# computablelabs/starks

Measured on AMD Instinct MI355X. Metric: ntt_field_elements_per_sec, higher is better.
Workload: dtype u256 (8 x u32 limbs, integer VALU)

## Files before the change

### starks_amd/csrc/ntt.hip

```cpp
#include <stdlib.h>

#include <atomic>

#include "knobs.hpp"
#include "ntt_kernels.cuh"

namespace {

template <int LOG_R, bool LAST, int TILE_LOG>
hipError_t launch_tile(const NttPassArgs& a, bool xcd, hipStream_t st) {
  constexpr int LOG_T = TILE_LOG - LOG_R;
  static std::atomic<uint64_t> attr_done{0};
  return shk_launch_tile_kernel(ntt_pass_kernel<LOG_R, LOG_T, LAST>, attr_done, LOG_T, 1u << (TILE_LOG - 2), (size_t)32 << TILE_LOG,
                                a, xcd, st);
}

template <int LOG_R, bool LAST, int TILE_LOG>
hipError_t launch_narrow(const NttPassArgs& a, hipStream_t st) {
  constexpr int LOG_T = TILE_LOG - LOG_R;
  const uint64_t tiles = (a.total + ((1ull << LOG_T) - 1)) >> LOG_T;
  if (tiles == 0 || tiles > 0x7ffffff0ull) return hipErrorInvalidValue;
  hipLaunchKernelGGL((ntt_narrow_pass_kernel<LOG_R, LOG_T, LAST>), dim3((unsigned)tiles), dim3(1u << (TILE_LOG - 1)), 0, st, a);
  return hipGetLastError();
}

template <int LOG_R, bool LAST>
hipError_t launch_cell(const ShkNttCell& c, const NttPassArgs& a, hipStream_t st) {
  if (c.form == SHK_NTT_NARROW) {
    if (c.xcd) return hipErrorInvalidValue;
    if constexpr (shk_ntt_cell_exists(SHK_NTT_NARROW, 10, LOG_R)) {
      if (c.tile_log == 10) return launch_narrow<LOG_R, LAST, 10>(a, st);
    }
    if constexpr (shk_ntt_cell_exists(SHK_NTT_NARROW, 9, LOG_R)) {
      if (c.tile_log == 9) return launch_narrow<LOG_R, LAST, 9>(a, st);
    }
    return hipErrorInvalidValue;
  }
  if constexpr (shk_ntt_cell_exists(SHK_NTT_TILE, 12, LOG_R)) {
    if (c.tile_log == 12) return launch_tile<LOG_R, LAST, 12>(a, c.xcd, st);
  }
  if constexpr (shk_ntt_cell_exists(SHK_NTT_TILE, 11, LOG_R)) {
    if (c.tile_log == 11) return launch_tile<LOG_R, LAST, 11>(a, c.xcd, st);
  }
  if constexpr (shk_ntt_cell_exists(SHK_NTT_TILE, 10, LOG_R)) {
    if (c.tile_log == 10) return launch_tile<LOG_R, LAST, 10>(a, c.xcd, st);
  }
  if constexpr (shk_ntt_cell_exists(SHK_NTT_TILE, 9, LOG_R)) {
    if (c.tile_log == 9) return launch_tile<LOG_R, LAST, 9>(a, c.xcd, st);
  }
  return hipErrorInvalidValue;
}

template <bool LAST>
hipError_t dispatch(const ShkNttCell& c, int log_R, const NttPassArgs& a, hipStream_t st) {
  switch (log_R) {
    case 2: return launch_cell<2, LAST>(c, a, st);
    case 3: return launch_cell<3, LAST>(c, a, st);
    case 4: return launch_cell<4, LAST>(c, a, st);
    case 5: return launch_cell<5, LAST>(c, a, st);
    case 6: return launch_cell<6, LAST>(c, a, st);
    case 7: return launch_cell<7, LAST>(c, a, st);
    case 8: return launch_cell<8, LAST>(c, a, st);
    case 9: return launch_cell<9, LAST>(c, a, st);
    case 10: return launch_cell<10, LAST>(c, a, st);
    case 11: return launch_cell<11, LAST>(c, a, st);
    default: return hipErrorInvalidValue;
  }
}

}

hipError_t shk_launch_ntt_cell(const ShkNttCell& c, int log_R, bool last, const NttPassArgs& a, hipStream_t st) {
  if (!shk_ntt_cell_exists(c.form, c.tile_log, log_R)) return hipErrorInvalidValue;
  return last ? dispatch<true>(c, log_R, a, st) : dispatch<false>(c, log_R, a, st);
}

hipError_t shk_launch_ntt_pass(int log_R, bool last, const NttPassArgs& a, hipStream_t st) {
  const ShkNttPassShape shape{a.total, a.log_n, a.log_S, a.pass_index};
  const ShkNttCell c = shk_ntt_choose_cell(shk_knobs(), log_R, last, shape);
  if (c.form == SHK_NTT_NONE) return hipErrorInvalidValue;
  return shk_launch_ntt_cell(c, log_R, last, a, st);
}

hipError_t shk_launch_ntt_tiny(const fp* src, fp* dst, uint32_t n, uint32_t batch, const fp* scale, hipStream_t st) {
  if (batch == 0) return hipSuccess;
  hipLaunchKernelGGL(ntt_tiny_kernel, dim3((batch + 63) / 64), dim3(64), 0, st, src, dst, n, batch, scale);
  return hipGetLastError();
}
```

### starks_amd/csrc/ntt_kernels.cuh

```cuda
#pragma once
#include <stdlib.h>

#include <atomic>
#include <type_traits>

#include "internal.hpp"
#include "knobs.hpp"


__host__ __device__ constexpr uint32_t lds_slot(uint32_t e) {
  uint32_t s = (e ^ (e >> 3) ^ (e >> 6) ^ (e >> 9)) & 7u;
  return (((e >> 3) << 3) | s) * 2u;
}
__device__ __forceinline__ void lds_put_at(uint4* lds, uint32_t o, const fp& r) {
  lds[o] = make_uint4(r.v[0], r.v[1], r.v[2], r.v[3]);
  lds[o + 1] = make_uint4(r.v[4], r.v[5], r.v[6], r.v[7]);
}
__device__ __forceinline__ fp lds_get_at(const uint4* lds, uint32_t o) {
  uint4 a = lds[o], b = lds[o + 1];
  fp r;
  r.v[0] = a.x; r.v[1] = a.y; r.v[2] = a.z; r.v[3] = a.w;
  r.v[4] = b.x; r.v[5] = b.y; r.v[6] = b.z; r.v[7] = b.w;
  return r;
}
__device__ __forceinline__ void lds_put(uint4* lds, uint32_t e, const fp& r) {
  uint32_t o = lds_slot(e);
  lds[o] = make_uint4(r.v[0], r.v[1], r.v[2], r.v[3]);
  lds[o + 1] = make_uint4(r.v[4], r.v[5], r.v[6], r.v[7]);
}
__device__ __forceinline__ fp lds_get(const uint4* lds, uint32_t e) {
  uint32_t o = lds_slot(e);
  uint4 a = lds[o], b = lds[o + 1];
  fp r;
  r.v[0] = a.x; r.v[1] = a.y; r.v[2] = a.z; r.v[3] = a.w;
  r.v[4] = b.x; r.v[5] = b.y; r.v[6] = b.z; r.v[7] = b.w;
  return r;
}

__device__ __forceinline__ fp tw_lookup(const NttPassArgs& a, uint64_t e) {
  if (a.tw_direct) return fp_load(a.tw_lo + e);
  fp lo = fp_load(a.tw_lo + (e & ((1ull << a.tw_lb) - 1)));
  fp hi = fp_load(a.tw_hi + (e >> a.tw_lb));
  return fp_mul(lo, hi);
}

template <class F>
__device__ __forceinline__ void static_for4(F&& f) {
  f(std::integral_constant<int, 0>{});
  f(std::integral_constant<int, 1>{});
  f(std::integral_constant<int, 2>{});
  f(std::integral_constant<int, 3>{});
}

struct TileThread {
  fp x[4];
  uint32_t t, ibase;
  bool active;
  uint64_t gbase;
  uint64_t j2;
  uint64_t obase;
  uint64_t sbase;
};

#ifndef SHK_WAVE_LOCAL
#define SHK_WAVE_LOCAL 1
#endif
template <int LOG_R, int LOG_T>
__host__ __device__ constexpr bool tile_wave_local() {
  constexpr int LOG_W = LOG_R + LOG_T - 8;
  if (!SHK_WAVE_LOCAL || LOG_W < 0 || LOG_T > 5 || LOG_R < 4) return false;
  constexpr int GA = (LOG_W + 1) / 2;
  return LOG_W <= LOG_R - 2 * GA;
}
template <int LOG_R, int LOG_T, bool LAST>
__host__ __device__ constexpr int tile_phase(int g) {
  if (LAST && g == 0) return -1;
  if (!tile_wave_local<LOG_R, LOG_T>()) return 2 + g;
  constexpr int LOG_W = LOG_R + LOG_T - 8;
  return g < (LOG_W + 1) / 2 ? 0 : 1;
}
template <int LOG_R, int LOG_T, int g>
__host__ __device__ __forceinline__ uint32_t tile_ibase(uint32_t tid) {
  constexpr int beta = (LOG_R - 2 * (g + 1)) > 0 ? (LOG_R - 2 * (g + 1)) : 0;
  if constexpr (!tile_wave_local<LOG_R, LOG_T>()) {
    const uint32_t rest = tid >> LOG_T;
    return ((rest >> beta) << (beta + 2)) | (rest & ((1u << beta) - 1u));
  } else {
    constexpr int LOG_W = LOG_R + LOG_T - 8;
    constexpr int GA = (LOG_W + 1) / 2;
    constexpr int wlo = g < GA ? (LOG_R - 2 * GA) - LOG_W : LOG_R - LOG_W;
    const uint32_t lane_i = (tid & 63u) >> LOG_T, wave = tid >> 6;
    uint32_t i = 0;
    int nl = 0, nw = 0;
#pragma unroll
    for (int p = 0; p < LOG_R; ++p) {
      if (p == beta || p == beta + 1) continue;
      if (p >= wlo && p < wlo + LOG_W) {
        i |= ((wave >> nw) & 1u) << p;
        ++nw;
      } else {
        i |= ((lane_i >> nl) & 1u) << p;
        ++nl;
      }
    }
    return i;
  }
}

template <int LOG_R, int LOG_T, bool LAST, int g>
__host__ __device__ __forceinline__ void tile_thread_coords(uint32_t tid, uint32_t* t, uint32_t* ibase) {
  constexpr int beta = (LOG_R - 2 * (g + 1)) > 0 ? (LOG_R - 2 * (g + 1)) : 0;
  if constexpr (LAST && g == 0) {
    const uint32_t rest = tid & ((1u << LOG_R) / 4 - 1);
    *t = tid >> (LOG_R - 2);
    *ibase = ((rest >> beta) << (beta + 2)) | (rest & ((1u << beta) - 1u));
  } else {
    *t = tid & ((1u << LOG_T) - 1);
    *ibase = tile_ibase<LOG_R, LOG_T, g>(tid);
  }
}

template <int LOG_R, int LOG_T, bool LAST, int g>
__device__ __forceinline__ void ntt_group(const NttPassArgs& a, uint4* lds, TileThread& th, uint32_t tid, uint64_t tile0) {
  constexpr int R = 1 << LOG_R;
  constexpr int G = (LOG_R + 1) / 2;
  constexpr int beta = (LOG_R - 2 * (g + 1)) > 0 ? (LOG_R - 2 * (g + 1)) : 0;
  tile_thread_coords<LOG_R, LOG_T, LAST, g>(tid, &th.t, &th.ibase);

  if (g == 0 || (LAST && g == 1)) {
    const uint64_t col_raw = tile0 + th.t;
    th.active = col_raw < a.total;
    const uint64_t col = th.active ? col_raw : a.total - 1;
    if (LAST) {
      const uint64_t b = col >> a.log_P;
      const uint32_t pp = (uint32_t)(col & ((1ull << a.log_P) - 1));
      const uint32_t lr1 = a.ndig ? a.dig_log[0] : 0;
      const uint32_t k1 = pp & ((1u << lr1) - 1u);
      const uint32_t rst = pp >> lr1;
      const uint32_t p = (k1 << (a.log_P - lr1)) | rst;
      uint32_t sh = a.log_P, wl = 0, acc = 0;
#pragma unroll
      for (uint32_t d = 0; d < 3; ++d) {
        if (d < a.ndig) {
          sh -= a.dig_log[d];
          acc |= ((p >> sh) & ((1u << a.dig_log[d]) - 1u)) << wl;
          wl += a.dig_log[d];
        }
      }
      th.gbase = (b << a.log_n) + ((uint64_t)p << LOG_R);
      th.obase = (b << a.log_n) + acc;
      th.sbase = b * a.src_n;
    } else {
      th.j2 = col & ((1ull << a.log_S) - 1);
      th.gbase = ((col >> a.log_S) << (LOG_R + a.log_S)) + th.j2;
      th.sbase = (col >> a.log_S) * a.src_n;
    }
  }

  constexpr int qhi = LOG_R - 1 - 2 * g;
  auto tw_needed = [](int b) constexpr {
    const int q = qhi - (b >> 1), pr = b & 1;
    if (q <= 0) return false;
    const int lb = q - beta;
    const int hl = lb == 1 ? pr : 2 * pr;
    if (q == 1 && beta == 0) return (hl & 1) != 0;
    return true;
  };
  auto tw_load = [&](int b) {
    const int q = qhi - (b >> 1), pr = b & 1;
    const int lb = q - beta;
    const int hl = lb == 1 ? pr : 2 * pr;
    if (q == 1 && beta == 0) return fp2_load(a.wR + (R / 4));
    const uint32_t il = th.ibase | ((uint32_t)hl << beta);
    const uint32_t ex = (il & ((1u << q) - 1u)) << (LOG_R - 1 - q);
    return fp2_load(a.wR + ex);
  };
  constexpr int first_tw = tw_needed(0) ? 0 : tw_needed(1) ? 1 : tw_needed(2) ? 2 : tw_needed(3) ? 3 : 4;
  fp2 tw_cur, tw_nxt;
  if constexpr (first_tw < 4) tw_cur = tw_load(first_tw);

  bool sparse_done = false;
  if constexpr (g == 0 && !LAST && LOG_R >= 4) {
    if (a.src_n && a.src_n <= ((uint64_t)(R / 4) << a.log_S)) {
      sparse_done = true;
      const uint64_t off = ((uint64_t)th.ibase << a.log_S) + th.j2;
      const bool in = off < a.src_n;
      th.x[0] = th.x[1] = th.x[2] = th.x[3] = fp_zero();
      if (FP_ANY(in)) {
        fp x0 = fp_load(a.src + th.sbase + (in ? off : 0));
        const fp2 tw_b = tw_load(2), tw_c = tw_load(3);
#pragma unroll
        for (int w = 0; w < 8; ++w) x0.v[w] = in ? x0.v[w] : 0u;
        th.x[0] = x0;
        th.x[2] = fp_mul2(x0, tw_cur);
        th.x[1] = fp_mul2(x0, tw_b);
        th.x[3] = fp_mul2(th.x[2], tw_c);
      }
    }
  }

  if (sparse_done) {
  } else if (g == 0) {
    if (a.src_n) {
#pragma unroll
      for (int h = 0; h < 4; ++h) {
        const uint32_t i = th.ibase | ((uint32_t)h << beta);
        const uint64_t off = LAST ? (uint64_t)i : (((uint64_t)i << a.log_S) + th.j2);
        const bool in = off < a.src_n;
        fp v = fp_load(a.src + th.sbase + (in ? off : 0));
#pragma unroll
        for (int w = 0; w < 8; ++w) v.v[w] = in ? v.v[w] : 0u;
        th.x[h] = v;
      }
    } else {
#pragma unroll
      for (int h = 0; h < 4; ++h) {
        const uint32_t i = th.ibase | ((uint32_t)h << beta);
        th.x[h] = LAST ? fp_load(a.src + th.gbase + i) : fp_load(a.src + th.gbase + ((uint64_t)i << a.log_S));
      }
    }
  } else {
#pragma unroll
    for (int h = 0; h < 4; ++h)
      th.x[h] = lds_get_at(lds, lds_slot((th.ibase << LOG_T) | th.t) ^ lds_slot((uint32_t)h << (beta + LOG_T)));
  }

  if (!sparse_done) static_for4([&](auto bc) {
    constexpr int b = decltype(bc)::value;
    constexpr int q = qhi - (b >> 1), pr = b & 1;
    if constexpr (q >= 0) {
      constexpr int lb = q - beta;
      constexpr int hl = lb == 1 ? pr : 2 * pr;
      constexpr int hh = hl | (1 << lb);
      constexpr int nxt = (b < 1 && tw_needed(1)) ? 1 : (b < 2 && tw_needed(2)) ? 2 : (b < 3 && tw_needed(3)) ? 3 : 4;
      if constexpr (tw_needed(b) && nxt < 4) tw_nxt = tw_load(nxt);
      const fp s = fp_add(th.x[hl], th.x[hh]);
      fp d = fp_sub(th.x[hl], th.x[hh]);
      if constexpr (tw_needed(b)) {
        d = fp_mul2(d, tw_cur);
        if constexpr (nxt < 4) tw_cur = tw_nxt;
      }
      th.x[hl] = s;
      th.x[hh] = d;
    }
  });

  if (g < G - 1) {
#pragma unroll
    for (int h = 0; h < 4; ++h) {
      lds_put_at(lds, lds_slot((th.ibase << LOG_T) | th.t) ^ lds_slot((uint32_t)h << (beta + LOG_T)), th.x[h]);
    }
    if constexpr (tile_phase<LOG_R, LOG_T, LAST>(g) == tile_phase<LOG_R, LOG_T, LAST>(g + 1)) {
      __builtin_amdgcn_fence(__ATOMIC_RELEASE, "wavefront");
      __builtin_amdgcn_wave_barrier();
      __builtin_amdgcn_fence(__ATOMIC_ACQUIRE, "wavefront");
    } else {
      __syncthreads();
    }
  }
}

#ifndef SHK_NTT_MIN_WAVES
#define SHK_NTT_MIN_WAVES 4
#endif
template <int LOG_R, int LOG_T, bool LAST>
__device__ __forceinline__ void ntt_pass_body(const NttPassArgs& a) {
  static_assert(LOG_R >= 2 && LOG_R <= 11 && LOG_T >= 0 && LOG_R + LOG_T >= 8 && LOG_R + LOG_T <= 12, "unsupported tile");
  constexpr int G = (LOG_R + 1) / 2;
  extern __shared__ __attribute__((aligned(16))) uint4 lds[];
  const uint32_t tid = threadIdx.x;
  uint64_t tile = blockIdx.x;
  if (a.xcd_per) {
    tile = (uint64_t)(blockIdx.x & 7u) * a.xcd_per + (blockIdx.x >> 3);
    if ((tile << LOG_T) >= a.total) return;
  }
  const uint64_t tile0 = tile << LOG_T;
  TileThread th;
  th.t = 0; th.ibase = 0; th.active = false; th.gbase = 0; th.j2 = 0; th.obase = 0; th.sbase = 0;
  fp itw[4];
  auto itw_load = [&](int h) {
    const uint32_t i = tile_ibase<LOG_R, LOG_T, G - 1>(tid) | (uint32_t)h;
    const uint32_t k = __brev(i) >> (32 - LOG_R);
    return fp_load(a.tw2 + ((uint64_t)k << a.log_S) + th.j2);
  };
  auto itw_request = [&]() {
    if (!LAST && a.tw2) itw[0] = itw_load(0);
  };
  if constexpr (G == 1) {
    ntt_group<LOG_R, LOG_T, LAST, 0>(a, lds, th, tid, tile0);
    itw_request();
  } else {
    ntt_group<LOG_R, LOG_T, LAST, 0>(a, lds, th, tid, tile0);
    if constexpr (G == 2) itw_request();
    ntt_group<LOG_R, LOG_T, LAST, 1>(a, lds, th, tid, tile0);
    if constexpr (G > 2) {
      if constexpr (G == 3) itw_request();
      ntt_group<LOG_R, LOG_T, LAST, 2>(a, lds, th, tid, tile0);
    }
    if constexpr (G > 3) {
      if constexpr (G == 4) itw_request();
      ntt_group<LOG_R, LOG_T, LAST, 3>(a, lds, th, tid, tile0);
    }
    if constexpr (G > 4) {
      if constexpr (G == 5) itw_request();
      ntt_group<LOG_R, LOG_T, LAST, 4>(a, lds, th, tid, tile0);
    }
    if constexpr (G > 5) {
      if constexpr (G == 6) itw_request();
      ntt_group<LOG_R, LOG_T, LAST, 5>(a, lds, th, tid, tile0);
    }
  }

  if (!th.active) return;
#pragma unroll
  for (int h = 0; h < 4; ++h) {
    const uint32_t i = th.ibase | (uint32_t)h;
    const uint32_t k = __brev(i) >> (32 - LOG_R);
    if (LAST) {
      fp v = th.x[h];
      if (a.scale) v = fp_mul(v, fp_load(a.scale));
      fp_store(a.dst + th.obase + ((uint64_t)k << a.log_P), v);
    } else {
      if (a.tw2 && h + 1 < 4) itw[h + 1] = itw_load(h + 1);
      const fp tw = a.tw2 ? itw[h] : tw_lookup(a, th.j2 * k);
      fp v = fp_mul(th.x[h], tw);
      fp_store(a.dst + th.gbase + ((uint64_t)k << a.log_S), v);
    }
  }
}

template <int LOG_R, int LOG_T, bool LAST>
__global__ void __launch_bounds__(1 << (LOG_R + LOG_T - 2), SHK_NTT_MIN_WAVES) ntt_pass_kernel(NttPassArgs a) {
  ntt_pass_body<LOG_R, LOG_T, LAST>(a);
}

template <int LOG_R, int LOG_T, bool LAST>
__global__ void __launch_bounds__(1 << (LOG_R + LOG_T - 1)) ntt_narrow_pass_kernel(NttPassArgs a) {
  static_assert(LOG_R >= 2 && LOG_R <= 10 && LOG_T >= 0 && (LOG_R + LOG_T == 10 || LOG_R + LOG_T == 9), "1024- or 512-element tiles");
  __shared__ __attribute__((aligned(16))) uint4 lds[2 << (LOG_R + LOG_T)];
  constexpr int R = 1 << LOG_R;
  const uint32_t tid = threadIdx.x;
  const uint32_t t_in = LAST ? tid >> (LOG_R - 1) : tid & ((1u << LOG_T) - 1u);
  const uint32_t p_in = LAST ? tid & (R / 2 - 1) : tid >> LOG_T;
  const uint32_t t = tid & ((1u << LOG_T) - 1u), p = tid >> LOG_T;
  const uint64_t tile0 = (uint64_t)blockIdx.x << LOG_T;
  const uint64_t col_in = tile0 + t_in < a.total ? tile0 + t_in : a.total - 1;
  const bool active = tile0 + t < a.total;
  const uint64_t col = active ? tile0 + t : a.total - 1;
  uint64_t gbase_in, gbase = 0, obase = 0, sbase_in, j2 = 0;
  if (LAST) {
    auto row_of = [&](uint64_t c, uint64_t* bb) {
      *bb = c >> a.log_P;
      const uint32_t pp = (uint32_t)(c & ((1ull << a.log_P) - 1));
      const uint32_t lr1 = a.ndig ? a.dig_log[0] : 0;
      const uint32_t k1 = pp & ((1u << lr1) - 1u), rst = pp >> lr1;
      return (k1 << (a.log_P - lr1)) | rst;
    };
    uint64_t b_in, b_out;
    const uint32_t row_in = row_of(col_in, &b_in), row = row_of(col, &b_out);
    uint32_t sh = a.log_P, wl = 0, acc = 0;
#pragma unroll
    for (uint32_t d = 0; d < 3; ++d) {
      if (d < a.ndig) {
        sh -= a.dig_log[d];
        acc |= ((row >> sh) & ((1u << a.dig_log[d]) - 1u)) << wl;
        wl += a.dig_log[d];
      }
    }
    gbase_in = (b_in << a.log_n) + ((uint64_t)row_in << LOG_R);
    obase = (b_out << a.log_n) + acc;
    sbase_in = b_in * a.src_n;
  } else {
    j2 = col & ((1ull << a.log_S) - 1);
    gbase = ((col >> a.log_S) << (LOG_R + a.log_S)) + j2;
    gbase_in = gbase;
    sbase_in = (col >> a.log_S) * a.src_n;
  }
  auto fetch = [&](uint32_t i) {
    if (a.src_n) {
      const uint64_t off = LAST ? (uint64_t)i : (((uint64_t)i << a.log_S) + j2);
      const bool in = off < a.src_n;
      fp v = fp_load(a.src + sbase_in + (in ? off : 0));
#pragma unroll
      for (int w = 0; w < 8; ++w) v.v[w] = in ? v.v[w] : 0u;
      return v;
    }
    return LAST ? fp_load(a.src + gbase_in + i) : fp_load(a.src + gbase_in + ((uint64_t)i << a.log_S));
  };
  fp x0, x1;
  uint32_t i_lo = 0;
  auto tw_of = [&](int q) {
    const uint32_t half = 1u << q, pq = q == LOG_R - 1 ? p_in : p;
    const uint32_t il = ((pq >> q) << (q + 1)) | (pq & (half - 1u));
    return fp2_load(a.wR + ((il & (half - 1u)) << (LOG_R - 1 - q)));
  };
  fp2 tw_cur, tw_nxt;
  if constexpr (LOG_R >= 2) tw_cur = tw_of(LOG_R - 1);
#pragma unroll
  for (int q = LOG_R - 1; q >= 0; --q) {
    const uint32_t half = 1u << q;
    const uint32_t tq = q == LOG_R - 1 ? t_in : t, pq = q == LOG_R - 1 ? p_in : p;
    i_lo = ((pq >> q) << (q + 1)) | (pq & (half - 1u));
    const uint32_t i_hi = i_lo | half;
    const uint32_t s_lo = lds_slot((i_lo << LOG_T) | tq), s_hi = lds_slot((i_hi << LOG_T) | tq);
    fp u, v;
    if (q == LOG_R - 1) {
      u = fetch(i_lo);
      v = fetch(i_hi);
    } else {
      u = lds_get_at(lds, s_lo);
      v = lds_get_at(lds, s_hi);
    }
    if (q > 1) tw_nxt = tw_of(q - 1);
    x0 = fp_add(u, v);
    x1 = fp_sub(u, v);
    if (q > 0) {
      x1 = fp_mul2(x1, tw_cur);
      if (q > 1) tw_cur = tw_nxt;
      lds_put_at(lds, s_lo, x0);
      lds_put_at(lds, s_hi, x1);
      __syncthreads();
    }
  }
  if (!active) return;
#pragma unroll
  for (int h = 0; h < 2; ++h) {
    const uint32_t k = __brev(i_lo | (uint32_t)h) >> (32 - LOG_R);
    fp v = h ? x1 : x0;
    if (LAST) {
      if (a.scale) v = fp_mul(v, fp_load(a.scale));
      fp_store(a.dst + obase + ((uint64_t)k << a.log_P), v);
    } else {
      const fp tw = a.tw2 ? fp_load(a.tw2 + ((uint64_t)k << a.log_S) + j2) : tw_lookup(a, j2 * k);
      fp_store(a.dst + gbase + ((uint64_t)k << a.log_S), fp_mul(v, tw));
    }
  }
}


inline hipError_t shk_launch_tile_kernel(void (*k)(NttPassArgs), std::atomic<uint64_t>& attr_done, int log_t, unsigned threads,
                                         size_t lds_bytes, const NttPassArgs& a, bool xcd, hipStream_t st) {
  int dev = 0;
  hipError_t e = hipGetDevice(&dev);
  if (e != hipSuccess) return e;
  const uint64_t bit = 1ull << (dev & 63);
  if (!(attr_done.load(std::memory_order_acquire) & bit)) {
    e = hipFuncSetAttribute(reinterpret_cast<const void*>(k), hipFuncAttributeMaxDynamicSharedMemorySize, (int)lds_bytes);
    if (e != hipSuccess) return e;
    attr_done.fetch_or(bit, std::memory_order_release);
  }
  const uint64_t tiles = (a.total + ((1ull << log_t) - 1)) >> log_t;
  if (tiles == 0) return hipSuccess;
  if (tiles > 0x7ffffff0ull) return hipErrorInvalidValue;
  NttPassArgs b = a;
  uint64_t grid = tiles;
  b.xcd_per = 0;
  if (xcd) {
    b.xcd_per = (uint32_t)((tiles + 7) / 8);
    grid = 8ull * b.xcd_per;
  }
  hipLaunchKernelGGL(k, dim3((unsigned)grid), dim3(threads), lds_bytes, st, b);
  return hipGetLastError();
}

static __global__ void ntt_tiny_kernel(const fp* src, fp* dst, uint32_t n, uint32_t batch, const fp* scale) {
  uint32_t b = blockIdx.x * blockDim.x + threadIdx.x;
  if (b >= batch) return;
  if (n == 1) {
    fp_store(dst + b, fp_load(src + b));
    return;
  }
  fp x0 = fp_load(src + 2ull * b), x1 = fp_load(src + 2ull * b + 1);
  fp s = fp_add(x0, x1), d = fp_sub(x0, x1);
  if (scale) {
    fp sc = fp_load(scale);
    s = fp_mul(s, sc);
    d = fp_mul(d, sc);
  }
  fp_store(dst + 2ull * b, s);
  fp_store(dst + 2ull * b + 1, d);
}
```

Baseline: 13.52 billion.

## Stage per-pass twiddle table in LDS instead of global loads

For tile kernels with radix up to 2^9, the workgroup copies the twiddle table (w and w128 pairs) from global memory into extra LDS space at group 0, using a swizzled slot layout to avoid bank conflicts. Later twiddle reads then come from LDS instead of scattered global loads. The copy is issued before the data loads and finished with a barrier afterward, to overlap its latency. The cost is more LDS per workgroup, which could lower occupancy, plus one extra __syncthreads per tile.

```diff
diff --git a/starks_amd/csrc/ntt.hip b/starks_amd/csrc/ntt.hip
--- a/starks_amd/csrc/ntt.hip
+++ b/starks_amd/csrc/ntt.hip
@@ -11,8 +11,8 @@
 hipError_t launch_tile(const NttPassArgs& a, bool xcd, hipStream_t st) {
   constexpr int LOG_T = TILE_LOG - LOG_R;
   static std::atomic<uint64_t> attr_done{0};
-  return shk_launch_tile_kernel(ntt_pass_kernel<LOG_R, LOG_T, LAST>, attr_done, LOG_T, 1u << (TILE_LOG - 2), (size_t)32 << TILE_LOG,
-                                a, xcd, st);
+  return shk_launch_tile_kernel(ntt_pass_kernel<LOG_R, LOG_T, LAST>, attr_done, LOG_T, 1u << (TILE_LOG - 2),
+                                tile_lds_bytes<LOG_R, LOG_T>(), a, xcd, st);
 }
 
 template <int LOG_R, bool LAST, int TILE_LOG>
diff --git a/starks_amd/csrc/ntt_kernels.cuh b/starks_amd/csrc/ntt_kernels.cuh
--- a/starks_amd/csrc/ntt_kernels.cuh
+++ b/starks_amd/csrc/ntt_kernels.cuh
@@ -120,6 +120,60 @@
   }
 }
 
+template <int LOG_R, int g>
+__host__ __device__ constexpr bool tile_tw_needed(int b) {
+  constexpr int beta = (LOG_R - 2 * (g + 1)) > 0 ? (LOG_R - 2 * (g + 1)) : 0;
+  constexpr int qhi = LOG_R - 1 - 2 * g;
+  const int q = qhi - (b >> 1), pr = b & 1;
+  if (q <= 0) return false;
+  const int lb = q - beta;
+  const int hl = lb == 1 ? pr : 2 * pr;
+  if (q == 1 && beta == 0) return (hl & 1) != 0;
+  return true;
+}
+template <int LOG_R, int g>
+__host__ __device__ constexpr uint32_t tile_tw_exponent(int b, uint32_t ibase) {
+  constexpr int beta = (LOG_R - 2 * (g + 1)) > 0 ? (LOG_R - 2 * (g + 1)) : 0;
+  constexpr int qhi = LOG_R - 1 - 2 * g;
+  const int q = qhi - (b >> 1), pr = b & 1;
+  const int lb = q - beta;
+  const int hl = lb == 1 ? pr : 2 * pr;
+  if (q == 1 && beta == 0) return (1u << LOG_R) / 4;
+  const uint32_t il = ibase | ((uint32_t)hl << beta);
+  return (il & ((1u << q) - 1u)) << (LOG_R - 1 - q);
+}
+
+#ifndef SHK_TW_LDS
+#define SHK_TW_LDS 1
+#endif
+template <int LOG_R, int LOG_T>
+__host__ __device__ constexpr bool tile_tw_in_lds() {
+  constexpr int TILE_LOG = LOG_R + LOG_T;
+  if (!SHK_TW_LDS || LOG_R > 9 || TILE_LOG < 8 || TILE_LOG > 12) return false;
+  constexpr long wgs = (LOG_R >= 8 ? 16 : 20) >> (TILE_LOG - 8);
+  return ((32L << TILE_LOG) + (32L << LOG_R)) * wgs <= 160L * 1024;
+}
+template <int LOG_R, int LOG_T>
+__host__ __device__ constexpr size_t tile_lds_bytes() {
+  return ((size_t)32 << (LOG_R + LOG_T)) + (tile_tw_in_lds<LOG_R, LOG_T>() ? (size_t)32 << LOG_R : 0);
+}
+__host__ __device__ constexpr uint32_t tw_lds_key(uint32_t ex) { return (ex ^ (ex >> 3) ^ (ex >> 4)) & 15u; }
+__host__ __device__ constexpr uint32_t tw_lds_slot(uint32_t ex, uint32_t c) {
+  const uint32_t k = tw_lds_key(ex);
+  return ((((ex & ~3u) | (k & 3u)) << 2) | (c ^ (k >> 2)));
+}
+template <int LOG_R, int LOG_T>
+__host__ __device__ constexpr int tile_tw_fill_chunks() {
+  constexpr int chunks = 2 << LOG_R, threads = 1 << (LOG_R + LOG_T - 2);
+  return (chunks + threads - 1) / threads;
+}
+template <int LOG_R, int LOG_T>
+__host__ __device__ constexpr int tile_tw_fill_chunk(uint32_t tid, int k) {
+  constexpr uint32_t chunks = 2u << LOG_R, threads = 1u << (LOG_R + LOG_T - 2);
+  const uint32_t j = tid + (uint32_t)k * threads;
+  return ((uint32_t)(k + 1) * threads <= chunks || j < chunks) ? (int)j : -1;
+}
+
 template <int LOG_R, int LOG_T, bool LAST, int g>
 __device__ __forceinline__ void ntt_group(const NttPassArgs& a, uint4* lds, TileThread& th, uint32_t tid, uint64_t tile0) {
   constexpr int R = 1 << LOG_R;
@@ -158,26 +212,47 @@
   }
 
   constexpr int qhi = LOG_R - 1 - 2 * g;
-  auto tw_needed = [](int b) constexpr {
-    const int q = qhi - (b >> 1), pr = b & 1;
-    if (q <= 0) return false;
-    const int lb = q - beta;
-    const int hl = lb == 1 ? pr : 2 * pr;
-    if (q == 1 && beta == 0) return (hl & 1) != 0;
-    return true;
-  };
+  constexpr bool TWL = tile_tw_in_lds<LOG_R, LOG_T>();
+  auto tw_needed = [](int b) constexpr { return tile_tw_needed<LOG_R, g>(b); };
   auto tw_load = [&](int b) {
-    const int q = qhi - (b >> 1), pr = b & 1;
-    const int lb = q - beta;
-    const int hl = lb == 1 ? pr : 2 * pr;
-    if (q == 1 && beta == 0) return fp2_load(a.wR + (R / 4));
-    const uint32_t il = th.ibase | ((uint32_t)hl << beta);
-    const uint32_t ex = (il & ((1u << q) - 1u)) << (LOG_R - 1 - q);
-    return fp2_load(a.wR + ex);
+    const uint32_t ex = tile_tw_exponent<LOG_R, g>(b, th.ibase);
+    if constexpr (TWL) {
+      const uint4* tw = lds + (2u << (LOG_R + LOG_T));
+      const uint32_t o = tw_lds_slot(ex, 0);
+      const uint4 c0 = tw[o], c1 = tw[o ^ 1u], c2 = tw[o ^ 2u], c3 = tw[o ^ 3u];
+      fp2 r;
+      r.w.v[0] = c0.x; r.w.v[1] = c0.y; r.w.v[2] = c0.z; r.w.v[3] = c0.w;
+      r.w.v[4] = c1.x; r.w.v[5] = c1.y; r.w.v[6] = c1.z; r.w.v[7] = c1.w;
+      r.w128.v[0] = c2.x; r.w128.v[1] = c2.y; r.w128.v[2] = c2.z; r.w128.v[3] = c2.w;
+      r.w128.v[4] = c3.x; r.w128.v[5] = c3.y; r.w128.v[6] = c3.z; r.w128.v[7] = c3.w;
+      return r;
+    } else {
+      return fp2_load(a.wR + ex);
+    }
   };
   constexpr int first_tw = tw_needed(0) ? 0 : tw_needed(1) ? 1 : tw_needed(2) ? 2 : tw_needed(3) ? 3 : 4;
   fp2 tw_cur, tw_nxt;
-  if constexpr (first_tw < 4) tw_cur = tw_load(first_tw);
+  constexpr int FILL = tile_tw_fill_chunks<LOG_R, LOG_T>();
+  static_assert(!TWL || FILL == 1 || FILL == 2, "twiddle copy: one or two chunks per thread");
+  uint4 tw_fill0 = make_uint4(0, 0, 0, 0), tw_fill1 = tw_fill0;
+  if constexpr (TWL && g == 0) {
+    const uint4* src = reinterpret_cast<const uint4*>(a.wR);
+    const int j0 = tile_tw_fill_chunk<LOG_R, LOG_T>(tid, 0), j1 = tile_tw_fill_chunk<LOG_R, LOG_T>(tid, 1);
+    tw_fill0 = src[j0 < 0 ? 0 : j0];
+    if constexpr (FILL == 2) tw_fill1 = src[j1 < 0 ? 0 : j1];
+    __builtin_amdgcn_fence(__ATOMIC_SEQ_CST, "singlethread");
+  }
+  auto tw_fill_finish = [&]() {
+    uint4* tw = lds + (2u << (LOG_R + LOG_T));
+    const int j0 = tile_tw_fill_chunk<LOG_R, LOG_T>(tid, 0), j1 = tile_tw_fill_chunk<LOG_R, LOG_T>(tid, 1);
+    if (j0 >= 0) tw[tw_lds_slot((uint32_t)j0 >> 2, (uint32_t)j0 & 3u)] = tw_fill0;
+    if constexpr (FILL == 2) {
+      if (j1 >= 0) tw[tw_lds_slot((uint32_t)j1 >> 2, (uint32_t)j1 & 3u)] = tw_fill1;
+    }
+    __syncthreads();
+    if constexpr (first_tw < 4) tw_cur = tw_load(first_tw);
+  };
+  if constexpr (first_tw < 4 && !(TWL && g == 0)) tw_cur = tw_load(first_tw);
 
   bool sparse_done = false;
   if constexpr (g == 0 && !LAST && LOG_R >= 4) {
@@ -186,8 +261,13 @@
       const uint64_t off = ((uint64_t)th.ibase << a.log_S) + th.j2;
       const bool in = off < a.src_n;
       th.x[0] = th.x[1] = th.x[2] = th.x[3] = fp_zero();
+      fp x0 = fp_zero();
+      if constexpr (TWL) {
+        if (FP_ANY(in)) x0 = fp_load(a.src + th.sbase + (in ? off : 0));
+        tw_fill_finish();
+      }
       if (FP_ANY(in)) {
-        fp x0 = fp_load(a.src + th.sbase + (in ? off : 0));
+        if constexpr (!TWL) x0 = fp_load(a.src + th.sbase + (in ? off : 0));
         const fp2 tw_b = tw_load(2), tw_c = tw_load(3);
 #pragma unroll
         for (int w = 0; w < 8; ++w) x0.v[w] = in ? x0.v[w] : 0u;
@@ -212,12 +292,14 @@
         for (int w = 0; w < 8; ++w) v.v[w] = in ? v.v[w] : 0u;
         th.x[h] = v;
       }
+      if constexpr (TWL) tw_fill_finish();
     } else {
 #pragma unroll
       for (int h = 0; h < 4; ++h) {
         const uint32_t i = th.ibase | ((uint32_t)h << beta);
         th.x[h] = LAST ? fp_load(a.src + th.gbase + i) : fp_load(a.src + th.gbase + ((uint64_t)i << a.log_S));
       }
+      if constexpr (TWL) tw_fill_finish();
     }
   } else {
 #pragma unroll
```

Result: faster. 13.80 billion, median of 6 (+2.1%).
